# DoumanAsh/compu

Measured on AMD Instinct MI355X. Metric: decompressed GB/s (whole node), batched 64 KiB DEFLATE blocks; % HBM peak, higher is better.
Workload: dtype u8

## Files before the change

### compu_amd/csrc/inflate.hip

```cpp
#include <cstddef>
#include <cstdio>
#include <cstdlib>
#include <mutex>

#include "chip_internal.h"
#include "launch_slots.h"
#include "wave_checksums.h"

namespace chip {

typedef uint32_t u32x2 __attribute__((ext_vector_type(2)));
typedef uint32_t u32x4 __attribute__((ext_vector_type(4)));
typedef u32x4 u32x4_u __attribute__((aligned(1)));
typedef u32x4 u32x4_a4 __attribute__((aligned(4)));
template <typename T>
__device__ __forceinline__ GAS T *rdfirst_gptr(T *p)
{
    return (GAS T *)rdfirst_ptr(p);
}

#ifndef CHIP_PHASE_FN
#define CHIP_PHASE_FN __attribute__((always_inline))
#endif

#ifdef CHIP_STATS
#define STAT_DECL unsigned long long st_[24] = {0}; unsigned long long st_t0_ = 0
#define STAT_T0() (st_t0_ = __builtin_readcyclecounter())
#define STAT_ACC(i) do { unsigned long long n_ = __builtin_readcyclecounter(); st_[i] += n_ - st_t0_; st_t0_ = n_; } while (0)
#define STAT_ADD(i, v) (st_[i] += (unsigned long long)(v))
#define STAT_PARAM , unsigned long long *st_, unsigned long long &st_t0_
#define STAT_ARG , st_, st_t0_
#else
#define STAT_DECL
#define STAT_T0()
#define STAT_ACC(i)
#define STAT_ADD(i, v)
#define STAT_PARAM
#define STAT_ARG
#endif

enum : uint32_t { K_LIT = 0, K_LEN = 1, K_EOB = 2, K_BAD = 3 };
__device__ __forceinline__ constexpr uint32_t mk_entry(uint32_t cl, uint32_t eb, uint32_t kind, uint32_t base)
{
    return cl | (eb << 4) | (kind << 8) | (base << 16);
}

constexpr int LIT_ROOT = 9;
constexpr int DIST_ROOT = 8;
constexpr int CL_ROOT = 7;

constexpr uint32_t F_HALT = 1u << 15, F_INV = 1u << 25, F_LEN = 1u << 31;
constexpr uint32_t D_BAD = 1u << 10, D_LONG = 1u << 11;

__device__ __forceinline__ uint32_t make_final(uint32_t sym, uint32_t len)
{
    if (sym < 256) return len | (len << 10) | (sym << 16);
    if (sym == 256) return len | (len << 10) | F_HALT;
    if (sym >= 286) return len | (len << 10) | F_HALT | F_INV;
    const uint32_t s = sym - 257;
    uint32_t eb = 0, base = 3 + s;
    if (s == 28) base = 258;
    else if (s >= 8) {
        eb = (s >> 2) - 1;
        base = 3 + ((4 + (s & 3)) << eb);
    }
    return len | (eb << 5) | ((len + eb) << 10) | (base << 16) | F_LEN;
}
__device__ __forceinline__ uint32_t make_dist16(uint32_t sym, uint32_t len)
{
    if (sym >= 30) return len | D_BAD;
    if (sym < 4) return len | (sym << 8);
    return len | (((sym >> 1) - 1) << 4) | ((2 + (sym & 1)) << 8);
}

#ifndef CHIP_S_BITS
#define CHIP_S_BITS 320
#define CHIP_XT_BITS 1536
#define CHIP_XT_BITS_FIXED 3072
#define CHIP_ROW_TOKENS 256
#endif
constexpr uint32_t S_BITS = CHIP_S_BITS;
constexpr uint32_t XT_BITS = CHIP_XT_BITS;
#ifndef CHIP_XT_BITS_FIXED
#define CHIP_XT_BITS_FIXED CHIP_XT_BITS
#endif
constexpr uint32_t XT_BITS_FIXED = CHIP_XT_BITS_FIXED;
constexpr uint32_t ROW_TOKENS = CHIP_ROW_TOKENS;
static_assert(S_BITS % 32 == 0 && ROW_TOKENS % 4 == 0 && 64 * ROW_TOKENS < 65536, "geometry");
constexpr uint32_t SEG_WORDS = S_BITS / 32 + 1;
constexpr uint32_t SEG_SHIFT = 24;
constexpr uint32_t SEG_MAGIC = ((1u << SEG_SHIFT) + S_BITS - 1) / S_BITS;
constexpr bool seg_magic_ok()
{
    for (uint32_t x = 0; x < 64u * S_BITS + 4096u; x++)
        if (((x * SEG_MAGIC) >> SEG_SHIFT) != x / S_BITS) return false;
    return true;
}
static_assert(seg_magic_ok() && (64u * S_BITS + 4096u) * (uint64_t)SEG_MAGIC < (1ull << 32), "segment index by multiplication");
constexpr uint32_t WIN_DW = (31 + 64 * S_BITS + 48 + 96 + 31) / 32 + 3;
constexpr uint32_t HDR_IN_DW = 192;

constexpr size_t ROWS_WORDS = (size_t)64 * ROW_TOKENS;
static_assert(64ull * ROW_TOKENS * 258 < (1ull << 32), "count_tokens() sums a super-round's output lengths in 32 bits");
__device__ __forceinline__ uint32_t row_base(uint32_t l) { return (l >> 3) * (8u * ROW_TOKENS) + (l & 7u) * 4u; }
__device__ __forceinline__ uint32_t row_word(uint32_t k) { return k + (k >> 2) * 28u; }


struct HuffMeta {
    uint32_t limit15[16];
    uint32_t offs[16];
    uint32_t maxlen;
};

#ifndef CHIP_CHUNK_BYTES
#define CHIP_CHUNK_BYTES 2560
#endif
#ifndef CHIP_COPY_LANE_MAX
#define CHIP_COPY_LANE_MAX 32
#endif
constexpr uint32_t CHUNK_BYTES = CHIP_CHUNK_BYTES;
constexpr uint32_t COPY_LANE_MAX = CHIP_COPY_LANE_MAX;
constexpr uint32_t MQ_CAP = 128;
constexpr uint32_t IMG_WORDS = CHUNK_BYTES / 4 + 8;
constexpr uint32_t TOK_RING = 4;
static_assert(CHUNK_BYTES % 4 == 0 && CHUNK_BYTES >= 1024 && COPY_LANE_MAX % 16 == 0 && IMG_WORDS % 2 == 0, "geometry");

constexpr uint32_t FLUSH_BYTES = 4 * (IMG_WORDS + 2 * MQ_CAP + 64 * TOK_RING + 128 + 4);
constexpr uint32_t HDR_BYTES = 4 * HDR_IN_DW + 4 * (1 << CL_ROOT) + 80 + sizeof(HuffMeta) + 64 + 320 + 2 * 288 + 2 * 32 + 2 * sizeof(HuffMeta);
constexpr uint32_t PHASE_BYTES = 8 * WIN_DW > FLUSH_BYTES ? (8 * WIN_DW > HDR_BYTES ? 8 * WIN_DW : HDR_BYTES) : (FLUSH_BYTES > HDR_BYTES ? FLUSH_BYTES : HDR_BYTES);
#ifndef CHIP_LDS_BYTES
#define CHIP_LDS_BYTES 8960
#endif
constexpr uint32_t POOL_WORDS = (CHIP_LDS_BYTES - 2 * 512 - 2 * 256 - PHASE_BYTES) / 4;
constexpr uint32_t POOL_U16 = 2 * POOL_WORDS;

struct alignas(16) WaveLds {
    union {
        struct {
            uint32_t win[WIN_DW];
            uint32_t bm[WIN_DW];
        } w;
        struct {
            uint32_t inbuf[HDR_IN_DW];
            uint32_t cl_lut[1 << CL_ROOT];
            uint32_t cl_sorted[20];
            HuffMeta cl_h;
            uint32_t count[16];
            uint8_t lens[320];
            uint16_t lit_sorted[288];
            uint16_t dist_sorted[32];
            HuffMeta lit_h, dist_h;
        } hdr;
        struct {
            uint32_t out[IMG_WORDS];
            uint2 mq[MQ_CAP];
            uint32_t tok[64 * TOK_RING];
            uint32_t pk[128];
            uint32_t trash[4];
        } fl;
        uint32_t phase_words_[PHASE_BYTES / 4];
    };
    uint16_t lit_root[1 << LIT_ROOT];
    uint16_t dist_root[1 << DIST_ROOT];
    uint32_t pool[POOL_WORDS];
};
static_assert(sizeof(WaveLds) <= CHIP_LDS_BYTES, "the waves per CU that CHIP_LDS_BYTES stands for");
static_assert(POOL_WORDS >= 413 + 142, "the tables of any valid block fit");
#ifndef CHIP_EXP_ALLOW_SMALL_LDS
static_assert(sizeof(WaveLds) >= 2048 * 4, "wave_crc32 needs 8 KB");
#endif

__device__ __forceinline__ uint32_t canon_index(const HuffMeta &H, uint32_t x15, uint32_t &l)
{
    l = 1;
    if (x15 >= H.limit15[15]) return 0xffffffffu;
#pragma unroll
    for (int j = 1; j < 15; j++) l += (x15 >= H.limit15[j]) ? 1u : 0u;
    return H.offs[l] + ((x15 - H.limit15[l - 1]) >> (15 - l));
}

struct CanonLim {
    uint32_t lim[16];
};
__device__ __forceinline__ CanonLim canon_limits(const HuffMeta &H)
{
    CanonLim c;
#pragma unroll
    for (int j = 0; j < 16; j++) c.lim[j] = rdfirst(H.limit15[j]);
    return c;
}
template <int LO, int HI>
__device__ __forceinline__ uint32_t canon_index_in(const HuffMeta &H, const CanonLim &c, uint32_t x15, uint32_t &l)
{
    l = LO;
#pragma unroll
    for (int j = LO; j < HI; j++) l += (x15 >= c.lim[j]) ? 1u : 0u;
    return H.offs[l] + ((x15 - H.limit15[l - 1]) >> (15 - l));
}

template <typename SortedT, typename MakeT>
__device__ __forceinline__ int canon_prep(uint32_t *count, const uint8_t *lens, int n_, bool code_lengths, SortedT *sorted, HuffMeta &H, MakeT make)
{
    const uint32_t lane = lane_id();
    const int n = (int)rdfirst((uint32_t)n_);
    if (lane < 16) count[lane] = 0;
    WSYNC();
    for (int s = lane; s < n; s += 64) {
        uint32_t l = lens[s];
        if (l) atomicAdd(&count[l], 1u);
    }
    WSYNC();
    const uint32_t c = lane >= 1 && lane <= 15 ? count[lane] : 0u;
    const uint32_t cincl = wave_incl_scan(c);
    const uint32_t off = cincl - c;
    const uint32_t lim = wave_incl_scan(lane <= 15 ? c << (15u - (lane & 15u)) : 0u);
    const uint32_t present = (uint32_t)__ballot(c != 0);
    const uint32_t maxlen = present ? 31u - (uint32_t)__clz((int)present) : 0u;
    const bool over = __any(lane <= 15 && lim > 32768u);
    const int left = rdlane(lim, 15) < 32768u ? 1 : 0;
    uint32_t mynext = off;
    if (lane <= 15) {
        H.limit15[lane] = lim;
        H.offs[lane] = off;
    }
    if (lane == 0) H.maxlen = maxlen;
    WSYNC();
    if (maxlen == 0) return 1;
    if (over) return -1;
    if (left > 0 && (code_lengths || maxlen != 1)) return -1;
    for (int base = 0; base < n; base += 64) {
        int s = base + (int)lane;
        uint32_t l = s < n ? lens[s] : 0;
        for (uint32_t pm = present & 0xfffeu; pm; pm &= pm - 1u) {
            const uint32_t ll = (uint32_t)__builtin_ctz(pm);
            uint64_t m = __ballot(l == ll);
            uint32_t bp = rdlane(mynext, ll);
            if (l == ll) sorted[bp + __popcll(m & lanemask_lt())] = make((uint32_t)s, l);
            if (lane == ll) mynext += __popcll(m);
        }
    }
    WSYNC();
    return 0;
}

__device__ CHIP_PHASE_FN int build_cl_table(WaveLds &L)
{
    const uint32_t lane = lane_id();
    HuffMeta &H = L.hdr.cl_h;
    const int r = canon_prep(L.hdr.count, L.hdr.lens, 19, true, L.hdr.cl_sorted, H, [](uint32_t s, uint32_t l) { return mk_entry(l, 0, K_LIT, s); });
    if (r < 0) return -1;
    for (uint32_t idx = lane; idx < (1u << CL_ROOT); idx += 64) {
        uint32_t e = mk_entry(1, 0, K_LIT, 0);
        if (r == 0) {
            uint32_t l;
            const uint32_t ci = canon_index(H, __brev(idx) >> 17, l);
            e = ci == 0xffffffffu ? mk_entry(H.maxlen, 0, K_BAD, 0) : L.hdr.cl_sorted[ci];
        }
        L.hdr.cl_lut[idx] = e;
    }
    WSYNC();
    return 0;
}

__device__ CHIP_PHASE_FN int build_litlen(WaveLds &L, const uint8_t *lens, int n, uint32_t &used)
{
    const uint32_t lane = lane_id();
    HuffMeta &H = L.hdr.lit_h;
    uint16_t *const sorted = L.hdr.lit_sorted;
    const int r = canon_prep(L.hdr.count, lens, n, false, sorted, H, [](uint32_t s, uint32_t) { return (uint16_t)s; });
    if (r != 0) return -1;
    const CanonLim CL = canon_limits(H);
    const uint32_t lim_r = CL.lim[LIT_ROOT], top = CL.lim[15];
    const uint32_t nshort = rdfirst(H.offs[LIT_ROOT + 1 <= 15 ? LIT_ROOT + 1 : 15]);
    const uint32_t nsym = rdfirst(H.offs[15]) + rdfirst(L.hdr.count[15]);
    const uint32_t nfirst = rdfirst(H.maxlen) <= (uint32_t)LIT_ROOT ? nsym : nshort;
    if (nfirst + 1 > POOL_WORDS) return 1;
    for (uint32_t i = lane; i < nfirst; i += 64) {
        const uint32_t s = sorted[i];
        L.pool[i] = make_final(s, lens[s]);
    }
    const uint32_t bad_idx = nfirst;
    const uint32_t bad_e = rdfirst(H.maxlen) | (rdfirst(H.maxlen) << 10) | F_HALT | F_INV;
    if (lane == 0) L.pool[bad_idx] = bad_e;
    for (uint32_t idx = lane; idx < (1u << LIT_ROOT); idx += 64) {
        const uint32_t x15 = __brev(idx) >> 17;
        if (x15 >= top) L.lit_root[idx] = (uint16_t)(bad_idx << 5);
        else if (x15 < lim_r) {
            uint32_t l;
            L.lit_root[idx] = (uint16_t)(canon_index_in<1, LIT_ROOT>(H, CL, x15, l) << 5);
        }
    }
    used = nfirst + 1;
    if (top > lim_r) {
        constexpr uint32_t P = 1u << (15 - LIT_ROOT);
        const uint32_t np = (top - lim_r + P - 1) / P;
        for (uint32_t j0 = 0; j0 < np; j0 += 64) {
            const uint32_t j = j0 + lane;
            const bool have = j < np;
            const uint32_t xj = lim_r + j * P;
            uint32_t sb = 0;
            if (have) {
                uint32_t l;
                (void)canon_index_in<LIT_ROOT + 1, 15>(H, CL, xj + P < top ? xj + P - 1 : top - 1, l);
                sb = l - LIT_ROOT;
            }
            const uint32_t size = have ? (1u << sb) : 0u;
            const uint32_t incl = wave_incl_scan(size);
            const uint32_t off = used + incl - size;
            const uint32_t total = rdlane(incl, 63);
            if (used + total > POOL_WORDS) return 1;
            if (have) {
                for (uint32_t t = 0; t < size; t++) {
                    const uint32_t x15 = sb ? xj + ((__brev(t) >> (32 - sb)) << (15 - LIT_ROOT - sb)) : xj;
                    uint32_t l, e = bad_e;
                    if (x15 < top) {
                        const uint32_t s = sorted[canon_index_in<LIT_ROOT + 1, 15>(H, CL, x15, l)];
                        e = make_final(s, l);
                    }
                    L.pool[off + t] = e;
                }
                L.lit_root[__brev(xj >> (15 - LIT_ROOT)) >> (32 - LIT_ROOT)] = (uint16_t)((off << 5) | sb);
            }
            used += total;
        }
    }
    WSYNC();
    return 0;
}

__device__ CHIP_PHASE_FN int build_dist(WaveLds &L, const uint8_t *lens, int n, uint32_t used)
{
    const uint32_t lane = lane_id();
    HuffMeta &H = L.hdr.dist_h;
    uint16_t *const sorted = L.hdr.dist_sorted;
    const int r = canon_prep(L.hdr.count, lens, n, false, sorted, H, [](uint32_t s, uint32_t) { return (uint16_t)s; });
    if (r < 0) return -1;
    if (r == 1) {
        for (uint32_t idx = lane; idx < (1u << DIST_ROOT); idx += 64) L.dist_root[idx] = (uint16_t)(1u | D_BAD);
        WSYNC();
        return 0;
    }
    const CanonLim CL = canon_limits(H);
    const uint32_t lim_r = CL.lim[DIST_ROOT], top = CL.lim[15], maxlen = rdfirst(H.maxlen);
    uint16_t *const pool16 = (uint16_t *)L.pool;
    for (uint32_t idx = lane; idx < (1u << DIST_ROOT); idx += 64) {
        const uint32_t x15 = __brev(idx) >> 17;
        if (x15 >= top) L.dist_root[idx] = (uint16_t)(maxlen | D_BAD);
        else if (x15 < lim_r) {
            uint32_t l;
            const uint32_t s = sorted[canon_index_in<1, DIST_ROOT>(H, CL, x15, l)];
            L.dist_root[idx] = (uint16_t)make_dist16(s, l);
        }
    }
    if (top > lim_r) {
        constexpr uint32_t P = 1u << (15 - DIST_ROOT);
        const uint32_t np = (top - lim_r + P - 1) / P;
        uint32_t used16 = 0;
        for (uint32_t j0 = 0; j0 < np; j0 += 64) {
            const uint32_t j = j0 + lane;
            const bool have = j < np;
            const uint32_t xj = lim_r + j * P;
            uint32_t sb = 0;
            if (have) {
                uint32_t l;
                (void)canon_index_in<DIST_ROOT + 1, 15>(H, CL, xj + P < top ? xj + P - 1 : top - 1, l);
                sb = l - DIST_ROOT;
            }
            const uint32_t size = have ? (1u << sb) : 0u;
            const uint32_t incl = wave_incl_scan(size);
            const uint32_t total = rdlane(incl, 63);
            if (2 * used + used16 + total > POOL_U16) return 1;
            const uint32_t base16 = POOL_U16 - used16 - incl;
            if (have) {
                for (uint32_t t = 0; t < size; t++) {
                    const uint32_t x15 = sb ? xj + ((__brev(t) >> (32 - sb)) << (15 - DIST_ROOT - sb)) : xj;
                    uint32_t l, e = maxlen | D_BAD;
                    if (x15 < top) {
                        const uint32_t s = sorted[canon_index_in<DIST_ROOT + 1, 15>(H, CL, x15, l)];
                        e = make_dist16(s, l);
                    }
                    pool16[base16 + t] = (uint16_t)e;
                }
                L.dist_root[__brev(xj >> (15 - DIST_ROOT)) >> (32 - DIST_ROOT)] = (uint16_t)(D_LONG | sb | ((base16 & 127u) << 4) | ((base16 >> 7) << 12));
            }
            used16 += total;
        }
    }
    WSYNC();
    return 0;
}
struct InWin {
    const uint32_t *g32;
    uint32_t total_dw;
    uint32_t win0;
};


__device__ __forceinline__ void win_load(WaveLds &L, InWin &w, uint32_t dw_start)
{
    WSYNC();
    w.win0 = dw_start;
    constexpr uint32_t PER_LANE = (HDR_IN_DW + 63) / 64;
    uint32_t v[PER_LANE];
#pragma unroll
    for (uint32_t j = 0; j < PER_LANE; j++) {
        const uint32_t i = dw_start + 64u * j + lane_id();
        v[j] = i < w.total_dw ? w.g32[i] : 0u;
    }
#pragma unroll
    for (uint32_t j = 0; j < PER_LANE; j++) {
        const uint32_t k = 64u * j + lane_id();
        if (k < HDR_IN_DW) L.hdr.inbuf[k] = v[j];
    }
    WSYNC();
}

__device__ __forceinline__ void win_ensure(WaveLds &L, InWin &w, uint32_t pos, uint32_t span = 64)
{
    uint32_t d = pos >> 5;
    if (d < w.win0 || d + ((span + 62u) >> 5) + 1u > w.win0 + HDR_IN_DW) win_load(L, w, d);
}

__device__ __forceinline__ void win_bits(const WaveLds &L, const InWin &w, uint32_t pos, uint32_t &lo, uint32_t &hi)
{
    uint32_t D = (pos >> 5) - w.win0, sh = pos & 31;
    uint32_t d0 = L.hdr.inbuf[D], d1 = L.hdr.inbuf[D + 1], d2 = L.hdr.inbuf[D + 2];
    lo = __builtin_amdgcn_alignbit(d1, d0, sh);
    hi = __builtin_amdgcn_alignbit(d2, d1, sh);
}

__device__ __forceinline__ void win_bits_uniform(const WaveLds &L, const InWin &w, uint32_t pos, uint32_t &lo, uint32_t &hi)
{
    uint32_t l, h;
    win_bits(L, w, pos, l, h);
    lo = rdfirst(l);
    hi = rdfirst(h);
}

__device__ __forceinline__ uint32_t bfe(uint32_t v, uint32_t off, uint32_t width) { return __builtin_amdgcn_ubfe(v, off, width); }

__device__ int32_t parse_wrapper(LDS_AS uint32_t *tab, const uint8_t *gin, uint32_t avail, int32_t format, uint32_t &wrap, uint32_t &hdr)
{
    wrap = 0;
    hdr = 0;
    if (avail < 2) return CHIP_NEED_INPUT;
    const uint32_t b0 = gin[0], b1 = gin[1];
    const bool allow_gzip = format == CHIP_FMT_GZIP || format == CHIP_FMT_AUTO;
    const bool allow_zlib = format == CHIP_FMT_ZLIB || format == CHIP_FMT_AUTO;
    if (allow_gzip && b0 == 0x1f && b1 == 0x8b) {
        wrap = 2;
        if (avail < 4) return CHIP_NEED_INPUT;
        const uint32_t flg = gin[3];
        if (gin[2] != 8) return Z_DATA_ERROR;
        if (flg & 0xe0) return Z_DATA_ERROR;
        if (avail < 10) return CHIP_NEED_INPUT;
        uint32_t k = 10;
        if (flg & 4) {
            if (avail < k + 2) return CHIP_NEED_INPUT;
            uint32_t xlen = gin[k] | ((uint32_t)gin[k + 1] << 8);
            k += 2;
            if (avail - k < xlen) return CHIP_NEED_INPUT;
            k += xlen;
        }
        for (uint32_t bit = 8; bit <= 16; bit <<= 1) {
            if (!(flg & bit)) continue;
            for (;;) {
                uint32_t idx = k + lane_id();
                uint64_t z = __ballot(idx < avail && gin[idx] == 0);
                if (z) {
                    k += (uint32_t)__ffsll((long long)z);
                    break;
                }
                if (avail - k <= 64) return CHIP_NEED_INPUT;
                k += 64;
            }
        }
        if (flg & 2) {
            if (avail < k + 2) return CHIP_NEED_INPUT;
            uint32_t crc = wave_crc32(tab, gin, k);
            if ((crc & 0xffffu) != (gin[k] | ((uint32_t)gin[k + 1] << 8))) return Z_DATA_ERROR;
            k += 2;
        }
        hdr = k;
        return ST_RUNNING;
    }
    if (!allow_zlib) return Z_DATA_ERROR;
    if (((b0 << 8) | b1) % 31u) return Z_DATA_ERROR;
    if ((b0 & 15u) != 8) return Z_DATA_ERROR;
    if ((b0 >> 4) + 8 > 15) return Z_DATA_ERROR;
    wrap = 1;
    hdr = 2;
    if (b1 & 0x20) {
        if (avail < 6) return CHIP_NEED_INPUT;
        hdr = 6;
        return CHIP_NEED_DICT;
    }
    return ST_RUNNING;
}

struct __attribute__((packed)) U32u { uint32_t v; };
struct __attribute__((packed)) U16u { uint16_t v; };
struct __attribute__((packed)) U128u { uint32_t x, y, z, w; };
typedef LDS_AS uint8_t lds_u8;

__device__ void wave_copy_stored(uint8_t *gdst, const uint32_t *g32, uint32_t total_dw, uint32_t so, uint32_t n)
{
    const uint32_t lane = lane_id();
    const uint8_t *gsrc = (const uint8_t *)g32 + so;
    uint32_t head = (uint32_t)((16u - ((uintptr_t)gdst & 15u)) & 15u);
    if (head > n) head = n;
    if (lane < head) gdst[lane] = gsrc[lane];
    uint32_t done = head;
    const uint32_t body = (n - done) & ~15u;
    if (body) {
        uint4 *d16 = (uint4 *)(gdst + done);
        const U128u *s16 = (const U128u *)(gsrc + done);
        const uint32_t cnt = body >> 4;
        uint32_t i = lane;
#ifdef CHIP_STORED_NT_LD
#define CHIP_STORED_LD(p) __builtin_nontemporal_load(p)
#else
#define CHIP_STORED_LD(p) (*(p))
#endif
#ifndef CHIP_STORED_PLAIN_ST
#define CHIP_STORED_ST(v, p) __builtin_nontemporal_store(v, p)
#else
#define CHIP_STORED_ST(v, p) (*(p) = (v))
#endif
#ifndef CHIP_STORED_DEPTH
#define CHIP_STORED_DEPTH 2
#endif
        for (; i + 64u * (CHIP_STORED_DEPTH - 1) < cnt; i += 64u * CHIP_STORED_DEPTH) {
            u32x4 v[CHIP_STORED_DEPTH];
#pragma unroll
            for (int k = 0; k < CHIP_STORED_DEPTH; k++) v[k] = CHIP_STORED_LD((const u32x4_u *)(s16 + i + 64u * k));
#pragma unroll
            for (int k = 0; k < CHIP_STORED_DEPTH; k++) CHIP_STORED_ST(v[k], (u32x4 *)(d16 + i + 64u * k));
        }
        for (; i < cnt; i += 64u) {
            const U128u a = s16[i];
            d16[i] = make_uint4(a.x, a.y, a.z, a.w);
        }
        done += body;
    }
    const uint32_t tail = n - done;
    if (lane < tail) gdst[done + lane] = gsrc[done + lane];
    (void)total_dw;
}

__device__ __forceinline__ uint32_t small_mod(uint32_t off, uint32_t d)
{
    uint32_t q = (uint32_t)(((float)off + 0.5f) * __builtin_amdgcn_rcpf((float)d));
    return off - q * d;
}
struct ChunkLds {
    uint32_t *out;
    uint2 *mq;
    uint32_t *tok;
    lds_u8 *trash;
};

__device__ __forceinline__ ChunkLds chunk_lds(WaveLds &L)
{
    ChunkLds c;
    c.out = L.fl.out;
    c.mq = L.fl.mq;
    c.tok = L.fl.tok;
    c.trash = (lds_u8 *)L.fl.trash;
    return c;
}

__device__ __forceinline__ void lds_put(lds_u8 *d, lds_u8 *trash, const U128u &v, uint32_t n)
{
    ((LDS_AS U32u *)(n >= 4 ? d : trash))->v = v.x;
    ((LDS_AS U32u *)((n >= 8 ? d : trash) + 4))->v = v.y;
    ((LDS_AS U32u *)((n >= 12 ? d : trash) + 8))->v = v.z;
    ((LDS_AS U32u *)((n >= 16 ? d : trash) + 12))->v = v.w;
    const uint32_t w = n < 4 ? v.x : n < 8 ? v.y : n < 12 ? v.z : v.w;
    lds_u8 *const t = d + (n & 12u);
    const bool two = (n & 2u) != 0, one = (n & 1u) != 0;
    ((LDS_AS U16u *)(two ? t : trash))->v = (uint16_t)w;
    *(one ? (two ? t + 2 : t) : trash) = (uint8_t)(two ? w >> 16 : w);
}

__device__ __forceinline__ void copy_one_match(lds_u8 *img, const uint8_t *base, uint32_t mis, uint32_t x, uint32_t len, uint32_t dist)
{
    const uint32_t lane = lane_id();
    const int32_t sx = (int32_t)x - (int32_t)dist;
    for (uint32_t i = lane; i < len; i += 64) {
        const int32_t s = sx + (int32_t)(dist >= len ? i : small_mod(i, dist));
        uint8_t b = 0;
        if (s < (int32_t)mis) b = ((GAS const uint8_t *)base)[s];
        if (s >= (int32_t)mis) b = img[s];
        img[x + i] = b;
    }
    LSYNC();
}

struct Round {
    uint32_t x, len, dist;
    bool glob;
    U128u v0, v1;
};

__device__ __forceinline__ void round_issue(Round &r, const ChunkLds &C, const uint8_t *base, uint32_t mis, uint32_t qh, uint32_t nr,
                                            bool glob_ok)
{
    const uint32_t lane = lane_id();
    const bool act = lane < nr;
    const uint32_t qi = (qh + lane) & (MQ_CAP - 1u);
    const uint2 e = C.mq[qi];
    r.x = e.x;
    const uint32_t ld = act ? e.y : 0u;
    r.len = ld & 0xffffu;
    r.dist = ld >> 16;
    const int32_t sx = (int32_t)r.x - (int32_t)r.dist;
    r.glob = glob_ok && r.len != 0 && r.len <= COPY_LANE_MAX && sx + (int32_t)r.len <= (int32_t)mis;
    r.v0 = U128u{0, 0, 0, 0};
    r.v1 = U128u{0, 0, 0, 0};
#ifndef CHIP_EXP_NO_GLOB
    if (r.glob) {
        const u32x4_u t = *(GAS const u32x4_u *)(base + sx);
        r.v0 = U128u{t.x, t.y, t.z, t.w};
    }
#endif
#ifndef CHIP_EXP_NO_GLOB
    if (r.glob && r.len > 16u) {
        const u32x4_u t = *(GAS const u32x4_u *)(base + sx + 16);
        r.v1 = U128u{t.x, t.y, t.z, t.w};
    }
#endif
}

__device__ __forceinline__ void round_finish(const Round &r, const ChunkLds &C, const uint8_t *base, uint32_t mis STAT_PARAM)
{
    const uint32_t lane = lane_id();
    lds_u8 *const img = (lds_u8 *)C.out;
    const int32_t sx = (int32_t)r.x - (int32_t)r.dist;
    uint64_t pend = __ballot(r.len != 0);
    STAT_ADD(14, 1);
    while (pend) {
        const uint32_t f = (uint32_t)__ffsll((long long)pend) - 1u;
        const uint32_t wp = rdlane(r.x, f);
        const bool mine = (pend >> lane) & 1ull;
        const bool loc = sx >= (int32_t)mis && (uint32_t)sx + r.len <= wp;
        const bool ready = mine && r.len <= COPY_LANE_MAX && (r.glob || loc);
        const uint64_t rm = __ballot(ready);
        if (!((rm >> f) & 1ull)) {
            STAT_ADD(15, 1);
            copy_one_match(img, base, mis, wp, rdlane(r.len, f), rdlane(r.dist, f));
            pend &= pend - 1ull;
            continue;
        }
        STAT_ADD(12, 1);
        uint32_t rem = ready ? r.len : 0u;
#pragma unroll
        for (uint32_t it = 0; it < COPY_LANE_MAX / 16; it++) {
            if (it && !__any(rem != 0)) break;
            U128u v = it ? r.v1 : r.v0;
            if (rem && !r.glob) {
                const lds_u8 *sp = img + sx + (int32_t)(16u * it);
                v.x = ((const LDS_AS U32u *)sp)->v;
                v.y = ((const LDS_AS U32u *)(sp + 4))->v;
                v.z = ((const LDS_AS U32u *)(sp + 8))->v;
                v.w = ((const LDS_AS U32u *)(sp + 12))->v;
            }
            const uint32_t n = rem < 16u ? rem : 16u;
            lds_put(img + r.x + 16u * it, C.trash, v, n);
            rem -= n;
        }
        LSYNC();
        pend &= ~rm;
    }
}

__device__ __forceinline__ uint32_t lane_gather(uint32_t x, uint32_t src)
{
    return (uint32_t)__builtin_amdgcn_ds_bpermute((int)(src << 2), (int)x);
}

__device__ uint32_t token_end(const WaveLds &L, const InWin &w, uint32_t p)
{
    const uint16_t *const pool16 = (const uint16_t *)L.pool;
    const uint32_t i = p >> 5;
    const uint32_t d0 = i < w.total_dw ? w.g32[i] : 0u, d1 = i + 1u < w.total_dw ? w.g32[i + 1u] : 0u, d2 = i + 2u < w.total_dw ? w.g32[i + 2u] : 0u;
    const uint32_t lo = __builtin_amdgcn_alignbit(d1, d0, p), hi = __builtin_amdgcn_alignbit(d2, d1, p);
    const uint32_t r = L.lit_root[lo & ((1u << LIT_ROOT) - 1u)];
    const uint32_t e = L.pool[(r >> 5) + __builtin_amdgcn_ubfe(lo, LIT_ROOT, r)];
    const uint32_t n1 = __builtin_amdgcn_ubfe(e, 10, 5);
    if (!(e & F_LEN)) return p + n1;
    const uint32_t w2 = __builtin_amdgcn_alignbit(hi, lo, n1);
    uint32_t m = L.dist_root[w2 & ((1u << DIST_ROOT) - 1u)];
    if (m & D_LONG) {
        const uint32_t b16 = ((m >> 4) & 127u) | ((m >> 12) << 7);
        m = pool16[b16 + __builtin_amdgcn_ubfe(w2, DIST_ROOT, m)];
    }
    return p + n1 + (m & 15u) + __builtin_amdgcn_ubfe(m, 4, 4);
}

__device__ __attribute__((always_inline)) uint32_t overflow_bit(const WaveLds &L, const InWin &w, const uint32_t *grow, uint32_t ntok, uint32_t npieces,
                                                           uint32_t cstart, uint32_t run0, uint32_t xcap, uint32_t B)
{
    const uint32_t lane = lane_id();
    const uint32_t pfirst = lane < npieces ? L.fl.pk[2u * lane] : 0xffffffffu;
    const uint32_t pdelta = lane < npieces ? L.fl.pk[2u * lane + 1u] : 0u;
    uint32_t run = run0;
    for (uint32_t g = cstart; g < ntok; g += 64u) {
        const uint32_t t = g + lane < ntok ? g + lane : ntok - 1u;
        uint32_t k = 0;
        for (uint32_t q = 0; q < npieces; q++) k += rdlane(pfirst, q) <= t ? 1u : 0u;
        const uint32_t d = lane_gather(pdelta, k - 1u);
        const uint32_t krow = (t + d) & 0xffffu, rb = d >> 16;
        const uint32_t tok = grow[rb + row_word(krow)];
        uint32_t olen = (tok & 512u) ? (tok & 0x1ffu) : 1u;
        if (g + lane >= ntok) olen = 0;
        const uint32_t incl = wave_incl_scan(olen);
        const uint64_t over = __ballot(olen != 0 && run + incl > xcap);
        if (over) {
            const uint32_t f = (uint32_t)__ffsll((long long)over) - 1u;
            const uint32_t rbf = rdlane(rb, f), kf = rdlane(krow, f);
            const uint32_t owner = ((rbf / (8u * ROW_TOKENS)) << 3) | ((rbf % (8u * ROW_TOKENS)) >> 2);
            uint32_t p = B + owner * S_BITS;
            for (uint32_t j = 0; j <= kf; j++) p = rdfirst(token_end(L, w, p));
            return p;
        }
        run += rdlane(incl, 63u);
    }
    return 0;
}

__device__ CHIP_PHASE_FN bool flush_tokens(WaveLds &L, const uint32_t *grow_, uint32_t ntok_, uint32_t npieces_, uint8_t *gout_, uint32_t &opos_,
                             uint32_t cap_, int32_t &status, uint32_t (&ovf)[3] STAT_PARAM)
{
    const uint32_t lane = lane_id();
    const uint32_t *const grow = rdfirst_ptr(grow_);
    uint8_t *const gout = rdfirst_ptr(gout_);
    const uint32_t ntok = rdfirst(ntok_), npieces = rdfirst(npieces_), cap = rdfirst(cap_);
    uint32_t opos = rdfirst(opos_);
    const ChunkLds C = chunk_lds(L);
    lds_u8 *const img = (lds_u8 *)C.out;
    if (ntok == 0) return true;
    const uint32_t pfirst = lane < npieces ? L.fl.pk[2u * lane] : 0xffffffffu;
    const uint32_t pdelta = lane < npieces ? L.fl.pk[2u * lane + 1u] : 0u;
    uint32_t before = 0;
    uint32_t nfirst = 0;
    uint32_t dcur = 0;
    uint32_t gnext = 0;
    uint32_t slot_w = 0;
    const uint32_t tok_lds = rdfirst((uint32_t)(uintptr_t)(LDS_AS uint32_t *)C.tok);
    auto fetch = [&]() {
        const uint32_t g = gnext;
        uint32_t d = dcur;
        while (nfirst - g < 64u) {
            dcur = rdlane(pdelta, before);
            d = lane >= nfirst - g ? dcur : d;
            before++;
            const uint32_t nx = rdlane(pfirst, before & 63u);
            nfirst = before < npieces ? nx : 0xffffffffu;
        }
        const uint32_t t = min(g + lane, ntok - 1u);
        gnext = g + 64u;
        const uint32_t krow = (t + d) & 0xffffu;
        const uint32_t *src = grow + ((d >> 16) + row_word(krow));
        const uint32_t dst = tok_lds + 256u * slot_w;
        uint32_t keep;
        asm volatile("s_mov_b32 %0, m0\n\ts_mov_b32 m0, %2\n\ts_nop 0\n\tglobal_load_lds_dword %1, off\n\ts_mov_b32 m0, %0"
                     : "=&s"(keep)
                     : "v"(src), "s"(dst)
                     : "memory");
        slot_w = (slot_w + 1u) & (TOK_RING - 1u);
    };
    WSYNC();
    uint32_t c0 = 0;
    uint32_t slot_r = 0;
#pragma unroll
    for (uint32_t k = 0; k < TOK_RING; k++) fetch();
    bool fresh = true;
    uint32_t mis = 0, run = 0, nq = 0, qh = 0, prod0 = 0, cstart = 0;
    uint8_t *base = gout;
    bool glob_ok = false, inflight = false;
    Round R;
    for (;;) {
        if (fresh) {
            STAT_ADD(13, 1);
            mis = (uint32_t)((uintptr_t)(gout + opos) & 3u);
            base = gout + opos - mis;
            glob_ok = cap - opos >= 16u;
            run = mis;
            prod0 = opos - mis;
            nq = qh = 0;
            cstart = c0;
            fresh = false;
        }
        static_assert(TOK_RING == 4, "the wait below counts three younger ring loads");
        asm volatile("s_waitcnt vmcnt(3)" ::: "memory");
        const uint32_t t = C.tok[64u * slot_r + lane];
        const bool ismatch = (t & 512u) != 0;
        const uint32_t len = ismatch ? t & 0x1ffu : 0u;
        const uint32_t val = ismatch ? __builtin_amdgcn_ubfe(t, 10, 16) + 1u : t;
        const uint32_t left = ntok - c0;
        uint32_t olen = ismatch ? len : 1u;
        olen = lane < left ? olen : 0u;
        const uint32_t incl = wave_incl_scan(olen);
        const uint32_t start = run + incl - olen;
        const uint32_t total = rdlane(incl, 63u);
        const uint64_t lenm = __ballot(len != 0);
        uint32_t nacc;
        bool ending, too_far = false;
        if (left >= 64u && run + total <= CHUNK_BYTES && (opos >= 32768u || (__ballot(val > prod0 + start) & lenm) == 0)) {
            asm volatile("; the common group" ::: "memory");
            const uint32_t qi = __builtin_amdgcn_mbcnt_hi((uint32_t)(lenm >> 32), __builtin_amdgcn_mbcnt_lo((uint32_t)lenm, nq)) & (MQ_CAP - 1u);
            *(len == 0 ? img + start : C.trash) = (uint8_t)val;
            *(len != 0 ? &C.mq[qi] : (uint2 *)(uint8_t *)C.trash) = make_uint2(start, len | (val << 16));
            nq += (uint32_t)__popcll(lenm);
            c0 += 64u;
            run += total;
            nacc = 64u;
            ending = c0 >= ntok;
        } else {
            const uint32_t nvalid = left < 64u ? left : 64u;
            const uint64_t validm = nvalid == 64u ? ~0ull : (1ull << nvalid) - 1ull;
            const uint64_t nofit = __ballot(incl > CHUNK_BYTES - run) & validm;
            const uint64_t badm = __ballot(val > prod0 + start) & lenm & validm;
            const uint64_t stopm = nofit | badm;
            nacc = stopm ? (uint32_t)__ffsll((long long)stopm) - 1u : nvalid;
            too_far = stopm != 0 && ((badm & ~nofit) >> nacc) & 1ull;
            if (stopm && !too_far && run != mis) nacc = 0;
            if (lane < nacc && len == 0) img[start] = (uint8_t)val;
            const uint64_t mm = lenm & (nacc == 64u ? ~0ull : (1ull << nacc) - 1ull);
            if (lane < nacc && len != 0) {
                const uint32_t qi = __builtin_amdgcn_mbcnt_hi((uint32_t)(mm >> 32), __builtin_amdgcn_mbcnt_lo((uint32_t)mm, nq)) & (MQ_CAP - 1u);
                C.mq[qi] = make_uint2(start, len | (val << 16));
            }
            nq += (uint32_t)__popcll(mm);
            c0 += nacc;
            if (stopm) {
                if (nacc) run = rdlane(start, nacc);
            } else {
                run += total;
            }
            ending = stopm != 0 || c0 >= ntok;
        }
        LSYNC();
        STAT_ACC(16);
        if (nq - qh >= 64u || ending) {
            do {
                if (inflight) {
                    round_finish(R, C, base, mis STAT_ARG);
                    inflight = false;
                }
                const uint32_t pq = nq - qh;
                if (pq >= 64u || (ending && pq != 0)) {
                    const uint32_t nr = pq < 64u ? pq : 64u;
                    round_issue(R, C, base, mis, qh, nr, glob_ok);
                    qh += nr;
                    inflight = true;
                }
            } while (ending && inflight);
        }
        STAT_ACC(17);
        if (nacc == 64u) {
            fetch();
            slot_r = (slot_r + 1u) & (TOK_RING - 1u);
        } else if (nacc != 0 && c0 < ntok) {
            gnext = c0;
            before = (uint32_t)__popcll(__ballot(pfirst < c0));
            dcur = rdlane(pdelta, before - 1u);
            {
                const uint32_t nx = rdlane(pfirst, before & 63u);
                nfirst = before < npieces ? nx : 0xffffffffu;
            }
            asm volatile("s_waitcnt vmcnt(0)" ::: "memory");
            slot_r = slot_w = 0;
#pragma unroll
            for (uint32_t k = 0; k < TOK_RING; k++) fetch();
        }
        if (!ending) continue;
        const uint32_t xcap = cap - (opos - mis);
        {
            const uint32_t xe = run < xcap ? run : xcap;
            for (uint32_t xq = 4u * lane; xq < xe; xq += 256u) {
                const uint32_t wv = C.out[xq >> 2];
                if (xq >= mis && xq + 4u <= xe) {
                    *(GAS uint32_t *)(base + xq) = wv;
                } else {
#pragma unroll
                    for (int k = 0; k < 4; k++)
                        if (xq + k >= mis && xq + k < xe) ((GAS uint8_t *)base)[xq + k] = (uint8_t)(wv >> (8 * k));
                }
            }
        }
        WSYNC();
        STAT_ACC(18);
        opos += run - mis;
        opos_ = opos;
        const bool no_room = opos > cap || (too_far && opos == cap);
        if (no_room || too_far) {
            if (no_room) {
                opos_ = cap;
                ovf[0] = cstart;
                ovf[1] = mis;
                ovf[2] = xcap;
            }
            status = no_room ? CHIP_NEED_OUTPUT : Z_DATA_ERROR;
            return false;
        }
        if (c0 >= ntok) return true;
        fresh = true;
    }
}
constexpr size_t SCRATCH_WORDS = ROWS_WORDS;


enum : uint32_t { R_JOIN = 1, R_LIMIT = 2, R_EOB = 3, R_NEED_INPUT = 4, R_BAD = 5 };

__device__ CHIP_PHASE_FN uint32_t walk_round(WaveLds &L, const InWin &w, const uint32_t B_, const uint32_t end_bit_, uint32_t *rows_, const uint32_t xt_bits,
                                             uint32_t &ntok_out, uint32_t &term_why, uint32_t &term_pos STAT_PARAM)
{
    const uint32_t lane = lane_id();
    const uint32_t B = rdfirst(B_), end_bit = rdfirst(end_bit_);
    GAS const uint32_t *const g32 = rdfirst_gptr(w.g32);
    const uint32_t total_dw = rdfirst(w.total_dw);
    GAS uint32_t *const myrow = rdfirst_gptr(rows_) + row_base(lane);
    uint16_t *const pool16 = (uint16_t *)L.pool;
    const uint32_t D0 = B >> 5;
    WSYNC();
    {
        constexpr uint32_t PER_LANE = (WIN_DW + 63) / 64;
        uint32_t v[PER_LANE];
#pragma unroll
        for (uint32_t j = 0; j < PER_LANE; j++) {
            const uint32_t i = D0 + 64u * j + lane;
            v[j] = i < total_dw ? g32[i] : 0u;
        }
#pragma unroll
        for (uint32_t j = 0; j < PER_LANE; j++) {
            const uint32_t k = 64u * j + lane;
            if (k < WIN_DW) {
                L.w.win[k] = v[j];
                L.w.bm[k] = 0;
            }
        }
    }
    LSYNC();
    STAT_ACC(1);
    STAT_ADD(8, 1);
    const uint32_t s0 = B + lane * S_BITS;
    const uint32_t own_end = s0 + S_BITS;
    uint32_t hard = own_end + xt_bits;
    {
        const uint32_t sr_end = B + 64u * S_BITS;
        hard = hard < sr_end ? hard : sr_end;
        hard = hard < end_bit ? hard : end_bit;
    }
    const uint32_t wbase = 32u * D0;
    const uint32_t own_end_r = own_end - wbase, hard_r = hard - wbase;
    uint32_t q = s0 - wbase, tl = 0, nst = 0;
    uint32_t jb = 0, z = 0;
    bool run = s0 < end_bit;
    auto token = [&](uint32_t &tok) -> bool {
        const uint32_t p = q;
        const uint32_t a = (p >> 3) & ~3u;
        const uint32_t bit = 1u << (p & 31u);
        const uint32_t mine = p < own_end_r ? bit : 0u;
        const uint32_t old = atomicOr((uint32_t *)((uint8_t *)L.w.bm + a), mine);
        jb = old & (bit - mine);
        const uint32_t *wp = (const uint32_t *)((const uint8_t *)L.w.win + a);
        const uint32_t d0 = wp[0], d1 = wp[1], d2 = wp[2];
        const uint32_t lo = __builtin_amdgcn_alignbit(d1, d0, p), hi = __builtin_amdgcn_alignbit(d2, d1, p);
        const uint32_t r = L.lit_root[lo & ((1u << LIT_ROOT) - 1u)];
        const uint32_t e = L.pool[(r >> 5) + __builtin_amdgcn_ubfe(lo, LIT_ROOT, r)];
        const uint32_t n1 = __builtin_amdgcn_ubfe(e, 10, 5);
        const uint32_t msk = (uint32_t)((int32_t)e >> 31);
        const uint32_t w2 = __builtin_amdgcn_alignbit(hi, lo, n1);
        uint32_t m = L.dist_root[w2 & ((1u << DIST_ROOT) - 1u)] & msk;
        if (m & D_LONG) {
            const uint32_t b16 = ((m >> 4) & 127u) | ((m >> 12) << 7);
            m = pool16[b16 + __builtin_amdgcn_ubfe(w2, DIST_ROOT, m)];
        }
        const uint32_t cl2 = m & 15u, eb2 = __builtin_amdgcn_ubfe(m, 4, 4);
        const uint32_t dm1 = (__builtin_amdgcn_ubfe(m, 8, 2) << eb2) + __builtin_amdgcn_ubfe(w2, cl2, eb2);
        z = (e & (F_HALT | F_INV)) | (m & D_BAD);
        tl = n1 + cl2 + eb2;
        q = p + tl;
        if ((jb | z) != 0 || q > hard_r) return false;
        const uint32_t v = __builtin_amdgcn_ubfe(lo, e, e >> 5) + __builtin_amdgcn_ubfe(e, 16, 9);
        tok = (((dm1 << 10) | 512u) & msk) | v;
        nst++;
        return true;
    };
    bool full = false;
    while (__any(run)) {
        STAT_ADD(11, 1);
        uint32_t t4[4];
#pragma unroll
        for (int k = 0; k < 4; k++) asm volatile("" : "=v"(t4[k]));
        const uint32_t ng = nst;
        if (run) {
            if (nst + 4u > ROW_TOKENS) {
                run = false;
                full = true;
            } else {
                bool ok = token(t4[0]);
                if (ok) {
                    ok = token(t4[1]);
                    if (ok) {
                        ok = token(t4[2]);
                        if (ok) ok = token(t4[3]);
                    }
                }
                run = ok;
            }
        }
        if (nst > ng) *(GAS u32x4 *)(myrow + 8u * ng) = u32x4{t4[0], t4[1], t4[2], t4[3]};
    }
    const bool dropped = s0 < end_bit && !full;
    const uint32_t pn = q + wbase;
    const uint32_t p = pn - (dropped ? tl : 0u);
    uint32_t why = R_LIMIT;
    if (s0 < end_bit && !full) {
        if (jb) why = R_JOIN;
        else if (pn > end_bit) why = R_NEED_INPUT;
        else if (z) why = z == F_HALT ? (uint32_t)R_EOB : (uint32_t)R_BAD;
    }
    STAT_ADD(21, __popcll(__ballot(nst != 0)));
    STAT_ACC(2);
    const uint32_t rel = p - B;
    const uint32_t jl = why == R_JOIN ? (__umul24(rel, SEG_MAGIC) >> SEG_SHIFT) & 63u : lane;
    uint32_t a_join = 0;
    if (__any(why == R_JOIN)) {
        const uint32_t sj = B + jl * S_BITS;
        const uint32_t w0 = (sj >> 5) - D0;
        const uint32_t lo_cut = sj & 31u;
        const uint32_t nb = p - (sj & ~31u);
#pragma unroll
        for (uint32_t t = 0; t < SEG_WORDS; t++) {
            uint32_t mw = L.w.bm[w0 + t];
            if (t == 0) mw &= ~0u << lo_cut;
            const int32_t k = (int32_t)nb - 32 * (int32_t)t;
            const uint32_t keep = k <= 0 ? 0u : k >= 32 ? 0xffffffffu : (1u << k) - 1u;
            a_join += __popc(mw & keep);
        }
        if (why != R_JOIN) a_join = 0;
    }
    uint32_t node = 0;
    {
        uint32_t pw = jl;
#pragma unroll
        for (int r = 0; r < 6; r++) {
            const uint32_t nx = lane_gather(pw, node);
            if ((lane >> r) & 1u) node = nx;
            pw = lane_gather(pw, pw);
        }
    }
    const uint32_t prev = wave_shr1(node);
    const bool fresh = lane == 0 || node != prev;
    const uint32_t e_nst = lane_gather(nst, node);
    const uint32_t g_a0 = lane_gather(a_join, prev);
    const uint32_t e_a0 = lane == 0 ? 0u : g_a0;
    const uint32_t cnt = (fresh && e_nst > e_a0) ? e_nst - e_a0 : 0u;
    const uint32_t incl = wave_incl_scan(cnt);
    const uint64_t nonempty = __ballot(cnt != 0);
    WSYNC();
    if (cnt) {
        const uint32_t k = (uint32_t)__popcll(nonempty & lanemask_lt()), first = incl - cnt;
        L.fl.pk[2u * k] = first;
        L.fl.pk[2u * k + 1u] = ((e_a0 - first) & 0xffffu) | (row_base(node) << 16);
    }
    const uint32_t kz = rdlane(node, 63);
    term_why = rdlane(why, kz);
    term_pos = rdlane(p, kz);
    ntok_out = rdlane(incl, 63u);
    WSYNC();
    STAT_ACC(3);
    STAT_ADD(9, __popcll(nonempty));
    STAT_ADD(10, ntok_out);
    return (uint32_t)__popcll(nonempty);
}

__device__ CHIP_PHASE_FN bool count_tokens(WaveLds &L, const uint32_t *grow_, uint32_t ntok_, uint32_t npieces_, uint64_t &osize, int32_t &status)
{
    const uint32_t lane = lane_id();
    GAS const uint32_t *const grow = rdfirst_gptr(grow_);
    const uint32_t ntok = rdfirst(ntok_), npieces = rdfirst(npieces_);
    if (ntok == 0) return true;
    const bool have = lane < npieces;
    const uint32_t pfirst = have ? L.fl.pk[2u * lane] : ntok;
    const uint32_t pdelta = have ? L.fl.pk[2u * lane + 1u] : 0u;
    const uint32_t pnext = lane + 1u < npieces ? L.fl.pk[2u * lane + 2u] : ntok;
    const uint32_t k0 = (pfirst + pdelta) & 0xffffu;
    const uint32_t kend = k0 + (have ? pnext - pfirst : 0u);
    GAS const uint32_t *const row = grow + (pdelta >> 16);
    uint32_t sum = 0;
    for (uint32_t kq = k0 & ~3u; __any(kq < kend); kq += 4u) {
        if (kq < kend) {
            const u32x4 t = *(GAS const u32x4 *)(row + 8u * kq);
            const uint32_t t4[4] = {t.x, t.y, t.z, t.w};
#pragma unroll
            for (uint32_t j = 0; j < 4; j++)
                if (kq + j >= k0 && kq + j < kend) sum += (t4[j] & 512u) ? t4[j] & 0x1ffu : 1u;
        }
    }
    const uint32_t incl = wave_incl_scan(sum);
    const uint32_t olo = rdfirst((uint32_t)osize), ohi = rdfirst((uint32_t)(osize >> 32));
    if (ohi == 0 && olo < 32768u) {
        uint32_t at = olo + incl - sum, badat = 0xffffffffu;
        for (uint32_t kq = k0 & ~3u; __any(kq < kend); kq += 4u) {
            if (kq < kend) {
                const u32x4 t = *(GAS const u32x4 *)(row + 8u * kq);
                const uint32_t t4[4] = {t.x, t.y, t.z, t.w};
#pragma unroll
                for (uint32_t j = 0; j < 4; j++)
                    if (kq + j >= k0 && kq + j < kend) {
                        const bool ismatch = (t4[j] & 512u) != 0;
                        if (ismatch && __builtin_amdgcn_ubfe(t4[j], 10, 16) + 1u > at && badat == 0xffffffffu) badat = at;
                        at += ismatch ? t4[j] & 0x1ffu : 1u;
                    }
            }
        }
        const uint64_t badm = __ballot(badat != 0xffffffffu);
        if (badm) {
            osize = rdlane(badat, (uint32_t)__ffsll((long long)badm) - 1u);
            status = Z_DATA_ERROR;
            return false;
        }
    }
    osize = (((uint64_t)ohi << 32) | olo) + rdlane(incl, 63u);
    return true;
}

template <bool SIZES>
__device__ CHIP_PHASE_FN void decode_block(WaveLds &L, InWin &w, uint32_t &pos, const uint32_t end_bit, uint8_t *gout, uint32_t &opos,
                                           const uint32_t cap, int32_t &status, uint32_t *rows, const uint32_t xt_bits, const uint32_t eob_len,
                                           const uint32_t flags, uint64_t &osize STAT_PARAM)
{
    pos = rdfirst(pos);
    opos = rdfirst(opos);
    for (;;) {
        if (pos >= end_bit) {
            status = CHIP_NEED_INPUT;
            return;
        }
        STAT_T0();
        uint32_t ntok = 0, why = 0, tpos = 0;
        const uint32_t npk = walk_round(L, w, pos, end_bit, rows, xt_bits, ntok, why, tpos STAT_ARG);
        int32_t st2 = ST_RUNNING;
        bool flushed = true;
        uint32_t ovf[3] = {0, 0, 0};
#ifdef CHIP_EXP_NO_FLUSH
        asm volatile("" ::"s"(npk), "s"(ntok));
#else
        if constexpr (SIZES) {
            if (npk) flushed = count_tokens(L, rows, ntok, npk, osize, st2);
        } else {
            if (npk) flushed = flush_tokens(L, rows, ntok, npk, gout, opos, cap, st2, ovf STAT_ARG);
        }
#endif
        w.win0 = 0xffffffffu;
        STAT_ACC(20);
        if (!flushed) {
            status = st2;
            if (!SIZES && (flags & F_COMPU_STATUS) && st2 == CHIP_NEED_OUTPUT) pos = overflow_bit(L, w, rows, ntok, npk, ovf[0], ovf[1], ovf[2], pos);
            return;
        }
        if (why == R_NEED_INPUT) {
            status = CHIP_NEED_INPUT;
            return;
        }
        if (why == R_EOB) {
            pos = tpos + eob_len;
            return;
        }
        if (why != R_LIMIT || tpos <= pos) {
            status = Z_DATA_ERROR;
            return;
        }
        pos = tpos;
    }
}

#ifndef CHIP_WAVES_PER_SIMD
#define CHIP_WAVES_PER_SIMD 5
#endif
template <bool SIZES>
__device__ __attribute__((always_inline)) void inflate_unit(const BatchArgs &a, const uint32_t u, WaveLds &L, uint32_t *scratch, uint64_t *out_size)
{
    const uint32_t lane = lane_id();

    const uint8_t *gin = a.in_base + a.in_off[u];
    const uint32_t in_len = a.in_len[u];
    uint8_t *gout = nullptr;
    uint32_t cap_ = 0xffffffffu;
    if constexpr (!SIZES) {
        gout = a.out_base + a.out_off[u];
        cap_ = a.out_cap[u];
    }
    const uint32_t cap = cap_;
    uint64_t osize = 0;

    InWin w;
    const uint32_t mis = (uint32_t)((uintptr_t)gin & 3u);
    w.g32 = (const uint32_t *)(gin - mis);
    w.total_dw = (mis + in_len + 3u) >> 2;
    w.win0 = 0xffffffffu;
    const uint32_t start_bit = mis * 8u;
    const uint32_t end_bit = start_bit + in_len * 8u;

    uint32_t pos = start_bit;
    uint32_t opos = 0;
    int32_t status = ST_RUNNING;
    bool last = false;
    int tables = 0;
    uint32_t eob_len = 0;

    STAT_DECL;
    STAT_T0();
    uint32_t wrap = 0;
    int32_t format = a.format;
    uint32_t ck_bit = 0, ck_opos = 0;
    bool resumed = false;
    uint32_t run_check = 0, run_cov = 0, out_dropped = 0;
    if (!SIZES && a.resume) {
        const uint32_t *rs = a.resume + RESUME_WORDS * u;
        const uint32_t r0 = rs[0], r1 = rs[1], r2 = rs[2];
        if (r0 != 0 && r0 <= in_len * 8u && r1 <= cap) {
            resumed = true;
            pos = start_bit + r0;
            opos = r1;
            wrap = r2 & 3u;
            ck_bit = r0;
            ck_opos = r1;
            run_check = rs[3];
            run_cov = rs[4];
            out_dropped = rs[5];
        }
    }
    if (!resumed && format != CHIP_FMT_DEFLATE) {
        uint32_t hdr = 0;
        status = parse_wrapper((LDS_AS uint32_t *)&L, gin, in_len, format, wrap, hdr);
        status = (int32_t)rdfirst((uint32_t)status);
        wrap = rdfirst(wrap);
        pos += rdfirst(hdr) * 8u;
    }
    if (status == ST_RUNNING) win_load(L, w, pos >> 5);

    __builtin_amdgcn_s_setprio(2);
    while (status == ST_RUNNING) {
        if (last) {
            status = CHIP_FINISHED;
            break;
        }
        ck_bit = pos - start_bit;
        ck_opos = opos;
        win_ensure(L, w, pos);
        if (pos + 3 > end_bit) {
            status = CHIP_NEED_INPUT;
            break;
        }
        uint32_t lo, hi;
        win_bits_uniform(L, w, pos, lo, hi);
        last = lo & 1u;
        uint32_t type = (lo >> 1) & 3u;
        pos += 3;
        if (type == 0) {
            pos = (pos + 7u) & ~7u;
            if (pos + 32 > end_bit) {
                status = CHIP_NEED_INPUT;
                break;
            }
            win_ensure(L, w, pos);
            win_bits_uniform(L, w, pos, lo, hi);
            uint32_t blen = lo & 0xffffu, nlen = lo >> 16;
            if (blen != (nlen ^ 0xffffu)) {
                status = Z_DATA_ERROR;
                break;
            }
            pos += 32;
            uint32_t avail = (end_bit - pos) >> 3;
            uint32_t ncopy = blen < avail ? blen : avail;
            if constexpr (SIZES) {
                osize += ncopy;
            } else {
                uint32_t room = cap - opos;
                if (ncopy > room) ncopy = room;
                wave_copy_stored(gout + opos, w.g32, w.total_dw, pos >> 3, ncopy);
                opos += ncopy;
            }
            pos += ncopy * 8u;
            if (ncopy < blen) {
                status = ncopy == avail ? CHIP_NEED_INPUT : CHIP_NEED_OUTPUT;
                break;
            }
            continue;
        }
        if (type == 3) {
            status = Z_DATA_ERROR;
            break;
        }
        uint32_t nlen = 288, ndist = 32;
        bool build = true;
        if (type == 1) {
            if (tables != 1) {
                for (uint32_t s = lane; s < 320; s += 64) L.hdr.lens[s] = s < 144 ? 8 : s < 256 ? 9 : s < 280 ? 7 : s < 288 ? 8 : 5;
                WSYNC();
                tables = 1;
            } else build = false;
        } else {
            tables = 2;
            if (pos + 14 > end_bit) {
                status = CHIP_NEED_INPUT;
                break;
            }
            win_ensure(L, w, pos);
            win_bits_uniform(L, w, pos, lo, hi);
            nlen = (lo & 31u) + 257;
            ndist = ((lo >> 5) & 31u) + 1;
            const uint32_t ncode = ((lo >> 10) & 15u) + 4;
            pos += 14;
            if (nlen > 286 || ndist > 30) {
                status = Z_DATA_ERROR;
                break;
            }
            if (pos + 3 * ncode > end_bit) {
                status = CHIP_NEED_INPUT;
                break;
            }
            win_ensure(L, w, pos, 128);
            if (lane < 19) L.hdr.lens[lane] = 0;
            WSYNC();
            if (lane < ncode) {
                static const uint8_t order[19] = {16, 17, 18, 0, 8, 7, 9, 6, 10, 5, 11, 4, 12, 3, 13, 2, 14, 1, 15};
                uint32_t l2, h2;
                win_bits(L, w, pos + 3 * lane, l2, h2);
                L.hdr.lens[order[lane]] = (uint8_t)(l2 & 7u);
            }
            WSYNC();
            pos += 3 * ncode;
            if (build_cl_table(L)) {
                status = Z_DATA_ERROR;
                break;
            }
            uint32_t have = 0, total = nlen + ndist, prevlen = 0;
            win_ensure(L, w, pos, 316 * 14 + 160);
            for (uint32_t k = lane; k < 320; k += 64) L.hdr.lens[k] = 0;
            WSYNC();
            while (have < total) {
                const uint32_t bp = pos + lane;
                uint32_t lo, hi;
                win_bits(L, w, bp, lo, hi);
                const uint32_t e = L.hdr.cl_lut[lo & 127u];
                const uint32_t cl = e & 15u, sym = e >> 16;
                const uint32_t eb = sym < 16 ? 0u : sym == 16 ? 2u : sym == 17 ? 3u : 7u;
                const uint32_t tl = cl + eb;
                const uint32_t run = sym < 16 ? 1u : (sym == 18 ? 11u : 3u) + bfe(lo, cl, eb);
                const uint32_t nx = lane + tl;
                uint32_t nth = 0;
                {
                    uint32_t pw = nx < 64u ? nx : 64u;
#pragma unroll
                    for (int r = 0; r < 6; r++) {
                        const uint32_t g1 = lane_gather(pw, nth & 63u), g2 = lane_gather(pw, pw & 63u);
                        if ((lane >> r) & 1u) nth = nth < 64u ? g1 : 64u;
                        pw = pw < 64u ? g2 : 64u;
                    }
                }
                uint8_t *const onflag = (uint8_t *)L.hdr.count;
                if (lane < 16) L.hdr.count[lane] = 0;
                LSYNC();
                if (nth < 64u) onflag[nth] = 1;
                LSYNC();
                const bool on = onflag[lane] != 0;
                const uint32_t c = on ? run : 0u;
                const uint32_t incl = wave_incl_scan(c);
                const uint32_t start = have + incl - c;
                const bool need = on && start < total;
                uint32_t bad = 0;
                if (need && bp + tl > end_bit) bad = 1;
                else if (need && sym == 16 && start == 0) bad = 2;
                else if (need && sym >= 16 && start + run > total) bad = 2;
                const uint64_t badm = __ballot(bad != 0);
                const uint32_t fb = badm ? (uint32_t)__ffsll((long long)badm) - 1u : 64u;
                const bool ok = need && lane < fb;
                const uint32_t expl = sym < 16 ? sym : 0u;
                const uint32_t m = wave_incl_max_scan((ok && sym != 16) ? (((lane + 1u) << 8) | expl) : 0u);
                const uint32_t v = sym == 16 ? (m ? m & 0xffu : prevlen) : expl;
                if (ok && sym < 16) L.hdr.lens[start] = (uint8_t)sym;
                if (ok && sym == 16)
                    for (uint32_t j = 0; j < run; j++) L.hdr.lens[start + j] = (uint8_t)v;
                if (badm) {
                    status = rdlane(bad, fb) == 1 ? (int32_t)CHIP_NEED_INPUT : Z_DATA_ERROR;
                    break;
                }
                const uint64_t okm = __ballot(ok);
                const uint32_t lv = 63u - (uint32_t)__clzll((long long)okm);
                have = rdlane(start + run, lv);
                pos += lv + rdlane(tl, lv);
                prevlen = rdlane(v, lv);
            }
            if (status != ST_RUNNING) break;
            WSYNC();
            STAT_ACC(4);
            if (rdfirst(L.hdr.lens[256]) == 0) {
                status = Z_DATA_ERROR;
                break;
            }
        }
        if (build) {
            eob_len = rdfirst(L.hdr.lens[256]);
            uint32_t used = 0;
            const int r1 = build_litlen(L, L.hdr.lens, (int)nlen, used);
            const int r2 = r1 ? r1 : build_dist(L, L.hdr.lens + nlen, (int)ndist, used);
            if (r1 || r2) {
                status = Z_DATA_ERROR;
                break;
            }
            STAT_ACC(5);
        }
        STAT_ACC(0);
        __builtin_amdgcn_s_setprio(0);
// ... 275 lines not shown
```

Baseline: 307.8.

## Pack two consecutive literals into one token during Huffman decode

The token decoder now looks up a second literal right after a literal, when the first symbol is not a length code and no segment-boundary mark is crossed. It packs both bytes into a single token flagged by bit 31. Output-length accounting, the flush scatter, overflow bit recovery and the size-check pass all learn the two-byte literal token. This is meant to cut tokens per output byte, and with it the row traffic and per-token flush work in literal-heavy streams. The cost is an extra LDS table lookup and bitmap read on every literal decode, plus added complexity in boundary handling.

```diff
diff --git a/compu_amd/csrc/inflate.hip b/compu_amd/csrc/inflate.hip
--- a/compu_amd/csrc/inflate.hip
+++ b/compu_amd/csrc/inflate.hip
@@ -105,6 +105,7 @@
 __device__ __forceinline__ uint32_t row_base(uint32_t l) { return (l >> 3) * (8u * ROW_TOKENS) + (l & 7u) * 4u; }
 __device__ __forceinline__ uint32_t row_word(uint32_t k) { return k + (k >> 2) * 28u; }
 
+__device__ __forceinline__ uint32_t tok_olen(uint32_t t) { return (t & 512u) ? t & 0x1ffu : 1u + (t >> 31); }
 
 struct HuffMeta {
     uint32_t limit15[16];
@@ -679,7 +680,7 @@
     return (uint32_t)__builtin_amdgcn_ds_bpermute((int)(src << 2), (int)x);
 }
 
-__device__ uint32_t token_end(const WaveLds &L, const InWin &w, uint32_t p)
+__device__ uint32_t token_end(const WaveLds &L, const InWin &w, uint32_t p, bool second)
 {
     const uint16_t *const pool16 = (const uint16_t *)L.pool;
     const uint32_t i = p >> 5;
@@ -688,8 +689,12 @@
     const uint32_t r = L.lit_root[lo & ((1u << LIT_ROOT) - 1u)];
     const uint32_t e = L.pool[(r >> 5) + __builtin_amdgcn_ubfe(lo, LIT_ROOT, r)];
     const uint32_t n1 = __builtin_amdgcn_ubfe(e, 10, 5);
-    if (!(e & F_LEN)) return p + n1;
     const uint32_t w2 = __builtin_amdgcn_alignbit(hi, lo, n1);
+    if (!(e & F_LEN)) {
+        if (!second) return p + n1;
+        const uint32_t r2 = L.lit_root[w2 & ((1u << LIT_ROOT) - 1u)];
+        return p + n1 + __builtin_amdgcn_ubfe(L.pool[(r2 >> 5) + __builtin_amdgcn_ubfe(w2, LIT_ROOT, r2)], 10, 5);
+    }
     uint32_t m = L.dist_root[w2 & ((1u << DIST_ROOT) - 1u)];
     if (m & D_LONG) {
         const uint32_t b16 = ((m >> 4) & 127u) | ((m >> 12) << 7);
@@ -712,7 +717,7 @@
         const uint32_t d = lane_gather(pdelta, k - 1u);
         const uint32_t krow = (t + d) & 0xffffu, rb = d >> 16;
         const uint32_t tok = grow[rb + row_word(krow)];
-        uint32_t olen = (tok & 512u) ? (tok & 0x1ffu) : 1u;
+        uint32_t olen = tok_olen(tok);
         if (g + lane >= ntok) olen = 0;
         const uint32_t incl = wave_incl_scan(olen);
         const uint64_t over = __ballot(olen != 0 && run + incl > xcap);
@@ -720,8 +725,12 @@
             const uint32_t f = (uint32_t)__ffsll((long long)over) - 1u;
             const uint32_t rbf = rdlane(rb, f), kf = rdlane(krow, f);
             const uint32_t owner = ((rbf / (8u * ROW_TOKENS)) << 3) | ((rbf % (8u * ROW_TOKENS)) >> 2);
+            const bool both = rdlane(run + incl - 1u, f) <= xcap;
             uint32_t p = B + owner * S_BITS;
-            for (uint32_t j = 0; j <= kf; j++) p = rdfirst(token_end(L, w, p));
+            for (uint32_t j = 0; j <= kf; j++) {
+                const uint32_t tj = rdfirst(grow[rbf + row_word(j)]);
+                p = rdfirst(token_end(L, w, p, (tj >> 31) != 0 && (j < kf || both)));
+            }
             return p;
         }
         run += rdlane(incl, 63u);
@@ -799,7 +808,8 @@
         const uint32_t len = ismatch ? t & 0x1ffu : 0u;
         const uint32_t val = ismatch ? __builtin_amdgcn_ubfe(t, 10, 16) + 1u : t;
         const uint32_t left = ntok - c0;
-        uint32_t olen = ismatch ? len : 1u;
+        const bool pair = (int32_t)t < 0;
+        uint32_t olen = ismatch ? len : 1u + (t >> 31);
         olen = lane < left ? olen : 0u;
         const uint32_t incl = wave_incl_scan(olen);
         const uint32_t start = run + incl - olen;
@@ -811,6 +821,7 @@
             asm volatile("; the common group" ::: "memory");
             const uint32_t qi = __builtin_amdgcn_mbcnt_hi((uint32_t)(lenm >> 32), __builtin_amdgcn_mbcnt_lo((uint32_t)lenm, nq)) & (MQ_CAP - 1u);
             *(len == 0 ? img + start : C.trash) = (uint8_t)val;
+            *(pair ? img + start + 1u : C.trash) = (uint8_t)(t >> 16);
             *(len != 0 ? &C.mq[qi] : (uint2 *)(uint8_t *)C.trash) = make_uint2(start, len | (val << 16));
             nq += (uint32_t)__popcll(lenm);
             c0 += 64u;
@@ -827,6 +838,7 @@
             too_far = stopm != 0 && ((badm & ~nofit) >> nacc) & 1ull;
             if (stopm && !too_far && run != mis) nacc = 0;
             if (lane < nacc && len == 0) img[start] = (uint8_t)val;
+            if (lane < nacc && pair) img[start + 1u] = (uint8_t)(t >> 16);
             const uint64_t mm = lenm & (nacc == 64u ? ~0ull : (1ull << nacc) - 1ull);
             if (lane < nacc && len != 0) {
                 const uint32_t qi = __builtin_amdgcn_mbcnt_hi((uint32_t)(mm >> 32), __builtin_amdgcn_mbcnt_lo((uint32_t)mm, nq)) & (MQ_CAP - 1u);
@@ -978,14 +990,28 @@
             const uint32_t b16 = ((m >> 4) & 127u) | ((m >> 12) << 7);
             m = pool16[b16 + __builtin_amdgcn_ubfe(w2, DIST_ROOT, m)];
         }
+#ifndef CHIP_EXP_NO_PAIR
+        const uint32_t r2 = L.lit_root[w2 & ((1u << LIT_ROOT) - 1u)];
+        const uint32_t e2 = L.pool[(r2 >> 5) + __builtin_amdgcn_ubfe(w2, LIT_ROOT, r2)];
+        const uint32_t p2 = p + n1;
+        const uint32_t mk2 = *(const uint32_t *)((const uint8_t *)L.w.bm + ((p2 >> 3) & ~3u));
+#endif
         const uint32_t cl2 = m & 15u, eb2 = __builtin_amdgcn_ubfe(m, 4, 4);
         const uint32_t dm1 = (__builtin_amdgcn_ubfe(m, 8, 2) << eb2) + __builtin_amdgcn_ubfe(w2, cl2, eb2);
         z = (e & (F_HALT | F_INV)) | (m & D_BAD);
         tl = n1 + cl2 + eb2;
+#ifndef CHIP_EXP_NO_PAIR
+        const uint32_t n2 = __builtin_amdgcn_ubfe(e2, 10, 5);
+        const bool pair = ((e | e2) & (F_LEN | F_HALT)) == 0 && p2 + n2 <= hard_r && ((mk2 >> (p2 & 31u)) & 1u) == 0;
+        tl += pair ? n2 : 0u;
+        const uint32_t pr = pair ? (e2 & 0x00ff0000u) | 0x80000000u : 0u;
+#else
+        const uint32_t pr = 0;
+#endif
         q = p + tl;
         if ((jb | z) != 0 || q > hard_r) return false;
         const uint32_t v = __builtin_amdgcn_ubfe(lo, e, e >> 5) + __builtin_amdgcn_ubfe(e, 16, 9);
-        tok = (((dm1 << 10) | 512u) & msk) | v;
+        tok = (((dm1 << 10) | 512u) & msk) | v | pr;
         nst++;
         return true;
     };
@@ -1098,7 +1124,7 @@
             const uint32_t t4[4] = {t.x, t.y, t.z, t.w};
 #pragma unroll
             for (uint32_t j = 0; j < 4; j++)
-                if (kq + j >= k0 && kq + j < kend) sum += (t4[j] & 512u) ? t4[j] & 0x1ffu : 1u;
+                if (kq + j >= k0 && kq + j < kend) sum += tok_olen(t4[j]);
         }
     }
     const uint32_t incl = wave_incl_scan(sum);
@@ -1114,7 +1140,7 @@
                     if (kq + j >= k0 && kq + j < kend) {
                         const bool ismatch = (t4[j] & 512u) != 0;
                         if (ismatch && __builtin_amdgcn_ubfe(t4[j], 10, 16) + 1u > at && badat == 0xffffffffu) badat = at;
-                        at += ismatch ? t4[j] & 0x1ffu : 1u;
+                        at += tok_olen(t4[j]);
                     }
             }
         }
```

Measured after the change: 321.5 (median of 6 runs). 4.4% higher.
